# quentinll/pertrenderer

Hardware: AMD Instinct MI355X
Metric: rendered frames/sec + ms/backward, 256² img, 50 faces/px, 8 samples (higher is better)
Workload: dtype f32; 1 GPU; cfg2 pose-opt step: sphere_642 (1280 faces), 256x256, faces_per_pixel=50, Sr=Sa=8 Gaussian, sigma=1e-3 gamma=1e-2, blur=ln(1e4-1)*sigma, fwd + L2 loss (native) + bwd + Adam step on the pose (lr 5e-2); image_size=256, faces_per_pixel=50, nb_samples=8, rast_samples=8, batch=1, execution=graph, parallelism=single GPU

## Files before the change

pertrenderer_amd/csrc/pr_rast.hip:

```cpp
#include <cstdlib>
#include <type_traits>

#include <hip/hip_fp16.h>

#include "pr_common.h"

namespace pr {
namespace {

constexpr float kEps = 1e-8f;
constexpr int kTile = 4;

struct V2 {
  float x, y;
};

template <bool FAST = false>
PR_DEV float dv(float a, float b) {
  if constexpr (FAST) return a * __builtin_amdgcn_rcpf(b);
  else return a / b;
}

PR_DEV float edge_fn(V2 p, V2 a, V2 b) { return (p.x - a.x) * (b.y - a.y) - (p.y - a.y) * (b.x - a.x); }

// ... 256 lines not shown

template <bool PERSP, bool CLIP>
PR_DEV bool face_test(const FaceRec& r, V2 p, float blur, float& pz) {
  const bool inbox = !(p.x < r.c.y || p.x > r.c.z || p.y < r.c.w || p.y > r.d.x);
  float bc[3], d;
  bool inside;
  face_eval<PERSP, CLIP>(r, p, bc, pz, inside, d);
  return inbox && !(pz < 0.f) && (inside || d < blur);
}

PR_DEV float dist_margin(float4 ra, float4 rb, float ptile, float sqrt_blur, float blur) {
  const float m = fmaxf(fmaxf(fmaxf(fabsf(ra.x), fabsf(ra.y)), fmaxf(fabsf(ra.w), fabsf(rb.x))),
                        fmaxf(fmaxf(fabsf(rb.z), fabsf(rb.w)), ptile));
  const float delta = m * 0x1p-19f;
  return 4.f * sqrt_blur * delta + 2.f * delta * delta + blur * 0x1p-20f;
}

PR_DEV float seg_dist2_fast(V2 p, V2 a, float bax, float bay, float l2, V2 b) {
  const float bx = p.x - b.x, by = p.y - b.y;
  const float db = bx * bx + by * by;
  float t = (bax * (p.x - a.x) + bay * (p.y - a.y)) * __builtin_amdgcn_rcpf(l2);
  t = t < 0.f ? 0.f : (t > 1.f ? 1.f : t);
  const float qx = a.x + t * bax, qy = a.y + t * bay;
  const float dx = p.x - qx, dy = p.y - qy;
  const float ds = dx * dx + dy * dy;
  return l2 <= kEps ? db : ds;
}

PR_DEV bool face_maybe(const FaceRec& r, V2 p, float blur, float margin, float& dfast) {
  const bool inbox = !(p.x < r.c.y || p.x > r.c.z || p.y < r.c.w || p.y > r.d.x);
  const V2 v0{r.a.x, r.a.y}, v1{r.a.w, r.b.x}, v2{r.b.z, r.b.w};
  const float e0 = (p.x - v1.x) * r.e.w - (p.y - v1.y) * r.e.z;
  const float e1 = (p.x - v2.x) * r.f.y - (p.y - v2.y) * r.f.x;
  const float e2 = (p.x - v0.x) * r.e.y - (p.y - v0.y) * r.e.x;
  const bool pos = r.d.y > 0.f;
  const bool ins = e0 != 0.f && e1 != 0.f && e2 != 0.f && (e0 > 0.f) == pos && (e1 > 0.f) == pos &&
                   (e2 > 0.f) == pos;
  const float d01 = seg_dist2_fast(p, v0, r.e.x, r.e.y, r.d.z, v1);
  const float d02 = seg_dist2_fast(p, v0, -r.f.x, -r.f.y, r.f.z, v2);
  const float d12 = seg_dist2_fast(p, v1, r.e.z, r.e.w, r.d.w, v2);
  float d = d01 < d02 ? d01 : d02;
  d = d < d12 ? d : d12;
  dfast = d;
  return inbox && (ins || !(d > blur + margin));
}

template <bool CLIP>
PR_DEV bool face_test_kept(const FaceRec& r, V2 p, float blur, float margin, float dfast, float& pz) {
  const V2 v0{r.a.x, r.a.y}, v1{r.a.w, r.b.x}, v2{r.b.z, r.b.w};
  const float z0 = r.a.z, z1 = r.b.y, z2 = r.c.x;
  const float area = r.d.y;
  const float e0 = (p.x - v1.x) * r.e.w - (p.y - v1.y) * r.e.z;
  const float e1 = (p.x - v2.x) * r.f.y - (p.y - v2.y) * r.f.x;
  const float e2 = (p.x - v0.x) * r.e.y - (p.y - v0.y) * r.e.x;
  const float b[3] = {e0 / area, e1 / area, e2 / area};
  float bc[3];
  if constexpr (CLIP) {
    clip_fwd(b, bc);
  } else {
    bc[0] = b[0]; bc[1] = b[1]; bc[2] = b[2];
  }
  pz = bc[0] * z0 + bc[1] * z1 + bc[2] * z2;
  const bool inside = b[0] > 0.f && b[1] > 0.f && b[2] > 0.f;
  bool near = dfast < blur - margin;
  if (!inside && !near && !(dfast > blur + margin)) {
    const float d01 = seg_dist2_d(p, v0, r.e.x, r.e.y, r.d.z, v1);
    const float d02 = seg_dist2_d(p, v0, -r.f.x, -r.f.y, r.f.z, v2);
    const float d12 = seg_dist2_d(p, v1, r.e.z, r.e.w, r.d.w, v2);
    float d = d01 < d02 ? d01 : d02;
    d = d < d12 ? d : d12;
    near = d < blur;
  }
  return !(pz < 0.f) && (inside || near);
}

PR_DEV bool in_bbox(const FaceRec& r, V2 p) {
  return !(p.x < r.c.y || p.x > r.c.z || p.y < r.c.w || p.y > r.d.x);
}

#ifdef PR_RAST_PROFILE
constexpr unsigned kProfTiles = 1 << 16;
__device__ long long g_rast_prof[kProfTiles * 16];
#define PR_STAMP(i) (stamp[i] += (long long)__builtin_amdgcn_s_memtime() - t_, t_ = __builtin_amdgcn_s_memtime())
#else
#define PR_STAMP(i) ((void)0)
#endif

template <int SL> struct RastCfg {
  static constexpr int CAP = SL == 1 ? 512 : (SL == 2 ? 256 : 128);
#ifndef PR_RAST_G4
#define PR_RAST_G4 2
#endif
  static constexpr int G = SL == 1 ? 4 : (SL >= 4 ? PR_RAST_G4 : 2);
#ifndef PR_RAST_CH4
#define PR_RAST_CH4 16
#endif
  static constexpr int CH = SL >= 4 ? PR_RAST_CH4 : 64;
  static_assert(CAP <= 8 * 64, "suffix-min pass holds CAP / 64 <= 8 entries per lane");
};
#ifndef PR_RAST_QPAD
template <int SL> constexpr int rast_qpad() { return SL == 4 ? 1 : 0; }
#else
template <int SL> constexpr int rast_qpad() { return PR_RAST_QPAD; }
#endif
#ifndef PR_RAST_MERGE
#define PR_RAST_MERGE 1
#endif
#ifndef PR_RAST_FRAGC
#define PR_RAST_FRAGC 1
#endif
#ifndef PR_RAST_CULLU
#define PR_RAST_CULLU 16
#endif
constexpr int kCullU = PR_RAST_CULLU;
#ifndef PR_RAST_CHUNKU
#define PR_RAST_CHUNKU 16
#endif
constexpr int kChunkU = PR_RAST_CHUNKU;

template <int NT>
PR_DEV void bitonic_sort(float* key, int* val, int n2, int tid) {
  for (int k = 2; k <= n2; k <<= 1) {
    for (int j = k >> 1; j > 0; j >>= 1) {
      for (int i = tid; i < n2; i += NT) {
        const int ixj = i ^ j;
        if (ixj > i) {
          const bool up = (i & k) == 0;
          const float a = key[i], b = key[ixj];
          if ((a > b) == up) {
            key[i] = b; key[ixj] = a;
            const int t = val[i]; val[i] = val[ixj]; val[ixj] = t;
          }
        }
      }
      __syncthreads();
    }
  }
}

template <int E>
PR_DEV void wave_bitonic_sort(float (&key)[E], int (&val)[E], int lane) {
#pragma unroll
  for (int k = 2; k <= E * 64; k <<= 1) {
#pragma unroll
    for (int j = k >> 1; j > 0; j >>= 1) {
      if (j >= 64) {
        const int je = j >> 6;
#pragma unroll
        for (int e = 0; e < E; ++e) {
          const int pe = e ^ je;
          if (pe > e) {
            const bool up = ((e * 64 + lane) & k) == 0;
            const float a = key[e], b = key[pe];
            if ((a > b) == up) {
              key[e] = b; key[pe] = a;
              const int t = val[e]; val[e] = val[pe]; val[pe] = t;
            }
          }
        }
      } else {
#pragma unroll
        for (int e = 0; e < E; ++e) {
          const float ok = __shfl_xor(key[e], j);
          const int ov = __shfl_xor(val[e], j);
          const int i = e * 64 + lane;
          const bool up = (i & k) == 0, lower = (lane & j) == 0;
// ... 836 lines not shown
  gv[0] = g0; gv[1] = g1; gv[2] = g2;
}

PR_DEV void persp_bwd(const float b[3], float z0, float z1, float z2, const float go[3], float gb[3], float gz[3]) {
  const float t0 = b[0] * z1 * z2, t1 = z0 * b[1] * z2, t2 = z0 * z1 * b[2];
  const float s = t0 + t1 + t2;
  float gt[3];
  if (s > kEps) {
    const float is = __builtin_amdgcn_rcpf(s);
    const float dot = (go[0] * t0 + go[1] * t1 + go[2] * t2) * (is * is);
    gt[0] = go[0] * is - dot; gt[1] = go[1] * is - dot; gt[2] = go[2] * is - dot;
  } else {
    gt[0] = go[0] * 1e8f; gt[1] = go[1] * 1e8f; gt[2] = go[2] * 1e8f;
  }
  gb[0] = gt[0] * z1 * z2; gb[1] = gt[1] * z0 * z2; gb[2] = gt[2] * z0 * z1;
  gz[0] = gt[1] * b[1] * z2 + gt[2] * z1 * b[2];
  gz[1] = gt[0] * b[0] * z2 + gt[2] * z0 * b[2];
  gz[2] = gt[0] * b[0] * z1 + gt[1] * z0 * b[1];
}

PR_DEV void clip_bwd(const float b[3], const float go[3], float gb[3]) {
  const float w0 = b[0] > 0.f ? b[0] : 0.f, w1 = b[1] > 0.f ? b[1] : 0.f, w2 = b[2] > 0.f ? b[2] : 0.f;
  const float s = w0 + w1 + w2;
  float gw[3];
  if (s > 1e-5f) {
    const float is = __builtin_amdgcn_rcpf(s);
    const float dot = (go[0] * w0 + go[1] * w1 + go[2] * w2) * (is * is);
    gw[0] = go[0] * is - dot; gw[1] = go[1] * is - dot; gw[2] = go[2] * is - dot;
  } else {
    gw[0] = go[0] * 1e5f; gw[1] = go[1] * 1e5f; gw[2] = go[2] * 1e5f;
  }
  gb[0] = b[0] > 0.f ? gw[0] : 0.f;
  gb[1] = b[1] > 0.f ? gw[1] : 0.f;
  gb[2] = b[2] > 0.f ? gw[2] : 0.f;
}

PR_DEV void slot_grad(const PRRastArgs& a, V2 p, const float* v, int64_t o, float g[9]) {
  const V2 v0{v[0], v[1]}, v1{v[3], v[4]}, v2{v[6], v[7]};
  const float z0 = v[2], z1 = v[5], z2 = v[8];
  const bool persp = a.perspective_correct != 0, clip = a.clip_barycentric_coords != 0;
  const float gzb = a.grad_zbuf ? a.grad_zbuf[o] : 0.f;
  const float gd = a.grad_dists ? a.grad_dists[o] : 0.f;
  float gbu[3] = {0.f, 0.f, 0.f};
  if (a.grad_bary) { gbu[0] = a.grad_bary[o * 3]; gbu[1] = a.grad_bary[o * 3 + 1]; gbu[2] = a.grad_bary[o * 3 + 2]; }
  float bw[3], bp[3], bc[3];
  bary_fwd(p, v0, v1, v2, bw);
  if (persp) persp_fwd<true>(bw, z0, z1, z2, bp); else { bp[0] = bw[0]; bp[1] = bw[1]; bp[2] = bw[2]; }
  if (clip) clip_fwd<true>(bp, bc); else { bc[0] = bp[0]; bc[1] = bp[1]; bc[2] = bp[2]; }
  const bool inside = bp[0] > 0.f && bp[1] > 0.f && bp[2] > 0.f;
  V2 gdv[3];
  tri_dist2_bwd(p, v0, v1, v2, inside ? -gd : gd, gdv);
  float gsum[3] = {gbu[0] + gzb * z0, gbu[1] + gzb * z1, gbu[2] + gzb * z2};
  float gpp[3] = {gsum[0], gsum[1], gsum[2]};
  if (clip) clip_bwd(bp, gsum, gpp);
  float gw[3] = {gpp[0], gpp[1], gpp[2]};
  float gz[3] = {0.f, 0.f, 0.f};
  if (persp) persp_bwd(bw, z0, z1, z2, gpp, gw, gz);
  V2 gbv[3];
  bary_bwd(p, v0, v1, v2, gw, gbv);
  g[0] = gbv[0].x + gdv[0].x; g[1] = gbv[0].y + gdv[0].y; g[2] = gzb * bc[0] + gz[0];
  g[3] = gbv[1].x + gdv[1].x; g[4] = gbv[1].y + gdv[1].y; g[5] = gzb * bc[1] + gz[1];
  g[6] = gbv[2].x + gdv[2].x; g[7] = gbv[2].y + gdv[2].y; g[8] = gzb * bc[2] + gz[2];
}

PR_DEV void acc_edge(V2 p, V2 a, V2 b, float g, float* ga, float* gb) {
  ga[0] += g * (p.y - b.y); ga[1] += g * (b.x - p.x);
  gb[0] += g * (a.y - p.y); gb[1] += g * (p.x - a.x);
}

PR_DEV void acc_seg(V2 p, V2 a, V2 b, float g, float* ga, float* gb) {
  const float bax = b.x - a.x, bay = b.y - a.y;
  const float l2 = bax * bax + bay * bay;
  float t = 1.f;
  if (!(l2 <= kEps)) {
    t = (bax * (p.x - a.x) + bay * (p.y - a.y)) / l2;
    t = t < 0.f ? 0.f : (t > 1.f ? 1.f : t);
  }
  const float qx = (1.f - t) * a.x + t * b.x, qy = (1.f - t) * a.y + t * b.y;
  const float dx = qx - p.x, dy = qy - p.y;
  ga[0] += g * (1.f - t) * 2.f * dx; ga[1] += g * (1.f - t) * 2.f * dy;
  gb[0] += g * t * 2.f * dx;         gb[1] += g * t * 2.f * dy;
}

PR_DEV void slot_grad_exact(const PRRastArgs& a, V2 p, const float* v, int64_t o, float out[9]) {
  const V2 v0{v[0], v[1]}, v1{v[3], v[4]}, v2{v[6], v[7]};
  const float z0 = v[2], z1 = v[5], z2 = v[8];
  const bool persp = a.perspective_correct != 0, clip = a.clip_barycentric_coords != 0;
  const float gzb = a.grad_zbuf ? a.grad_zbuf[o] : 0.f;
  const float gd = a.grad_dists ? a.grad_dists[o] : 0.f;
  float gbu[3] = {0.f, 0.f, 0.f};
  if (a.grad_bary) { gbu[0] = a.grad_bary[o * 3]; gbu[1] = a.grad_bary[o * 3 + 1]; gbu[2] = a.grad_bary[o * 3 + 2]; }
  float bw[3], bp[3], bc[3];
  bary_fwd(p, v0, v1, v2, bw);
  if (persp) persp_fwd(bw, z0, z1, z2, bp); else { bp[0] = bw[0]; bp[1] = bw[1]; bp[2] = bw[2]; }
  if (clip) clip_fwd(bp, bc); else { bc[0] = bp[0]; bc[1] = bp[1]; bc[2] = bp[2]; }
  const bool inside = bp[0] > 0.f && bp[1] > 0.f && bp[2] > 0.f;
  float gv[3][2] = {{0.f, 0.f}, {0.f, 0.f}, {0.f, 0.f}};
  {
    const float g = inside ? -gd : gd;
    const float e01 = seg_dist2(p, v0, v1), e02 = seg_dist2(p, v0, v2), e12 = seg_dist2(p, v1, v2);
    if (e01 <= e02 && e01 <= e12) acc_seg(p, v0, v1, g, gv[0], gv[1]);
    else if (e02 <= e01 && e02 <= e12) acc_seg(p, v0, v2, g, gv[0], gv[2]);
    else acc_seg(p, v1, v2, g, gv[1], gv[2]);
  }
  const float gsum[3] = {gbu[0] + gzb * z0, gbu[1] + gzb * z1, gbu[2] + gzb * z2};
  float gpp[3] = {gsum[0], gsum[1], gsum[2]};
  if (clip) {
    const float w0 = bp[0] > 0.f ? bp[0] : 0.f, w1 = bp[1] > 0.f ? bp[1] : 0.f, w2 = bp[2] > 0.f ? bp[2] : 0.f;
    const float s = w0 + w1 + w2;
    float gw[3];
    if (s > 1e-5f) {
      const float dot = (gsum[0] * w0 + gsum[1] * w1 + gsum[2] * w2) / (s * s);
      gw[0] = gsum[0] / s - dot; gw[1] = gsum[1] / s - dot; gw[2] = gsum[2] / s - dot;
    } else {
      gw[0] = gsum[0] / 1e-5f; gw[1] = gsum[1] / 1e-5f; gw[2] = gsum[2] / 1e-5f;
    }
    gpp[0] = bp[0] > 0.f ? gw[0] : 0.f; gpp[1] = bp[1] > 0.f ? gw[1] : 0.f; gpp[2] = bp[2] > 0.f ? gw[2] : 0.f;
  }
  float gw[3] = {gpp[0], gpp[1], gpp[2]}, gzp[3] = {0.f, 0.f, 0.f};
  if (persp) {
    const float t0 = bw[0] * z1 * z2, t1 = z0 * bw[1] * z2, t2 = z0 * z1 * bw[2];
    const float s = t0 + t1 + t2;
    float gt[3];
    if (s > kEps) {
      const float dot = (gpp[0] * t0 + gpp[1] * t1 + gpp[2] * t2) / (s * s);
      gt[0] = gpp[0] / s - dot; gt[1] = gpp[1] / s - dot; gt[2] = gpp[2] / s - dot;
    } else {
      gt[0] = gpp[0] / kEps; gt[1] = gpp[1] / kEps; gt[2] = gpp[2] / kEps;
    }
    gw[0] = gt[0] * z1 * z2; gw[1] = gt[1] * z0 * z2; gw[2] = gt[2] * z0 * z1;
    gzp[0] = gt[1] * bw[1] * z2 + gt[2] * z1 * bw[2];
    gzp[1] = gt[0] * bw[0] * z2 + gt[2] * z0 * bw[2];
    gzp[2] = gt[0] * bw[0] * z1 + gt[1] * z0 * bw[1];
  }
  const float area = edge_fn(v2, v0, v1) + kEps;
  const float e0 = edge_fn(p, v1, v2), e1 = edge_fn(p, v2, v0), e2 = edge_fn(p, v0, v1);
  const float darea = -(gw[0] * e0 + gw[1] * e1 + gw[2] * e2) / (area * area);
  acc_edge(p, v1, v2, gw[0] / area, gv[1], gv[2]);
  acc_edge(p, v2, v0, gw[1] / area, gv[2], gv[0]);
  acc_edge(p, v0, v1, gw[2] / area, gv[0], gv[1]);
  gv[2][0] += darea * (v1.y - v0.y);
  gv[2][1] += darea * (v0.x - v1.x);
  acc_edge(v2, v0, v1, darea, gv[0], gv[1]);
#pragma unroll
  for (int i = 0; i < 3; ++i) {
    out[i * 3 + 0] = gv[i][0];
    out[i * 3 + 1] = gv[i][1];
    out[i * 3 + 2] = gzb * bc[i] + gzp[i];
  }
}

template <bool EXACT>
PR_DEV void slot_grad_any(const PRRastArgs& a, V2 p, const float* v, int64_t o, float g[9]) {
  if constexpr (EXACT) slot_grad_exact(a, p, v, o, g);
  else slot_grad(a, p, v, o, g);
}

__global__ void rast_bwd_keys_kernel(PRRastArgs a, uint32_t* keys, int64_t s0, int64_t n) {
  for (int64_t i = (int64_t)blockIdx.x * blockDim.x + threadIdx.x; i < n; i += (int64_t)gridDim.x * blockDim.x) {
    const int64_t o = s0 + i, pix = o / a.K;
    const bool valid = a.pix_count ? (int)(o - pix * a.K) < a.pix_count[pix] : true;
    const int64_t f = valid ? a.pix_to_face[o] : -1;
    keys[i] = f >= 0 ? (uint32_t)f : (uint32_t)a.F;
  }
}

__global__ void rast_bwd_sorted_grad_kernel(PRRastArgs a, const uint32_t* keys, const uint32_t* idx, float* vals,
                                            int64_t s0, int64_t n) {
  for (int64_t i = (int64_t)blockIdx.x * blockDim.x + threadIdx.x; i < n; i += (int64_t)gridDim.x * blockDim.x) {
    const uint32_t f = keys[i];
    if ((int64_t)f >= a.F) continue;
    const int64_t o = s0 + idx[i];
    const int64_t pix = o / a.K;
    const int col = (int)(pix % a.W), row = (int)((pix / a.W) % a.H);
    const V2 p{ndc(a.W - 1 - col, a.W, a.H), ndc(a.H - 1 - row, a.H, a.W)};
    float g[9];
    slot_grad_exact(a, p, a.face_verts + (int64_t)f * 9, o, g);
#pragma unroll
    for (int c = 0; c < 9; ++c) vals[i * 9 + c] = g[c];
  }
}

constexpr int kHash = 512;
constexpr int kBwdTile = 8;
constexpr int kBwdThreads = 256;
#ifndef PR_BWD_ENT
#define PR_BWD_ENT 512
#endif
constexpr int kBwdEnt = PR_BWD_ENT;
constexpr int kBwdFaces = 128;

template <int ROWS, bool EXACT>
__global__ void __launch_bounds__(kBwdThreads) rast_bwd_kernel(PRRastArgs a, int order) {
  constexpr int tile_rows = ROWS, TP = kBwdTile * ROWS;
  __shared__ int hkey[kHash];
  __shared__ int hfl[kHash];
  __shared__ int flist[kBwdFaces];
  __shared__ alignas(8) uint16_t M[kBwdFaces * TP];
  __shared__ float gbuf[9 * kBwdEnt];
  __shared__ int2 clist[kBwdEnt];
  __shared__ int ccount, nface;
  __shared__ float pxs[kBwdTile], pys[ROWS];
  __shared__ int pcnt[kBwdTile * ROWS];
  __shared__ int pstart[kBwdTile * ROWS + 1];
  const int tid = threadIdx.x, lane = tid & 63;
  const int K = a.K, H = a.H, W = a.W;
  const int n = blockIdx.z, col0 = blockIdx.x * kBwdTile;
  const int row0 = (order ? centre_out(blockIdx.y, gridDim.y) : (int)blockIdx.y) * tile_rows;
  const int ncols = min(kBwdTile, W - col0), nrows = min(tile_rows, H - row0);
  const int64_t tile_o = (((int64_t)n * H + row0) * W + col0) * K;
  const int64_t row_stride = (int64_t)W * K;
  for (int i = tid; i < kHash; i += kBwdThreads) hkey[i] = -1;
  for (int i = tid; i < kBwdFaces * TP; i += kBwdThreads) M[i] = 0xffff;
  if (tid < kBwdTile) pxs[tid] = ndc(W - 1 - min(col0 + tid, W - 1), W, H);
  if (tid >= 64 && tid < 64 + ROWS) pys[tid - 64] = ndc(H - 1 - min(row0 + tid - 64, H - 1), H, W);
  if (tid == 0) nface = 0;
  if (tid < TP) {
    const int r = tid / kBwdTile, c = tid - r * kBwdTile;
    pcnt[tid] = (r < nrows && c < ncols) ? (a.pix_count ? a.pix_count[((int64_t)n * H + row0 + r) * W + col0 + c] : K) : 0;
  }
  __syncthreads();
  if (tid == 0) {
    int acc_s = 0;
    for (int q = 0; q < TP; ++q) { pstart[q] = acc_s; acc_s += pcnt[q]; }
    pstart[TP] = acc_s;
  }
  __syncthreads();
  const int total = pstart[TP];
  float acc[9] = {0.f, 0.f, 0.f, 0.f, 0.f, 0.f, 0.f, 0.f, 0.f};
  for (int c0 = 0; c0 < total; c0 += kBwdEnt) {
    if (tid == 0) ccount = 0;
    __syncthreads();
    int64_t f[kBwdEnt / kBwdThreads];
    int pk[kBwdEnt / kBwdThreads];
#pragma unroll
    for (int u = 0; u < kBwdEnt / kBwdThreads; ++u) {
      const int i = c0 + u * kBwdThreads + tid;
      f[u] = -1;
      pk[u] = 0;
      if (i < total) {
        int q = 0;
#pragma unroll
        for (int step = TP / 2; step > 0; step >>= 1)
          if (pstart[q + step] <= i) q += step;
        const int k = i - pstart[q], r = q / kBwdTile, c = q - r * kBwdTile;
        pk[u] = (q << 16) | k;
        f[u] = a.pix_to_face[tile_o + r * row_stride + c * K + k];
      }
    }
#pragma unroll
    for (int u = 0; u < kBwdEnt / kBwdThreads; ++u) {
      const bool keep = f[u] >= 0;
      const uint64_t bal = __ballot(keep);
      if (bal == 0) continue;
      int off = 0;
      if (lane == 0) off = atomicAdd(&ccount, __popcll(bal));
      off = __shfl(off, 0);
      if (!keep) continue;
      const int fi = (int)f[u];
      clist[off + __popcll(bal & ((1ull << lane) - 1ull))] = make_int2(pk[u], fi);
      uint32_t h = ((uint32_t)fi * 2654435761u) & (kHash - 1);
      for (int probe = 0; probe < 32; ++probe) {
        const int cur = atomicCAS(&hkey[h], -1, fi);
        if (cur == -1) {
          const int fl = atomicAdd(&nface, 1);
          hfl[h] = fl;
          if (fl < kBwdFaces) flist[fl] = fi;
          break;
        }
        if (cur == fi) break;
        h = (h + 1) & (kHash - 1);
      }
    }
    __syncthreads();
    const int nv = ccount;
    for (int j = tid; j < nv; j += kBwdThreads) {
      const int2 e = clist[j];
      const int pix = e.x >> 16, k = e.x & 0xffff, fi = e.y;
      const int r = pix >> 3, c = pix & 7;
      const int64_t o = tile_o + r * row_stride + c * K + k;
      const V2 p{pxs[c], pys[r]};
      float g[9];
      slot_grad_any<EXACT>(a, p, a.face_verts + (int64_t)fi * 9, o, g);
      uint32_t h = ((uint32_t)fi * 2654435761u) & (kHash - 1);
      int fl = kBwdFaces;
      for (int probe = 0; probe < 32; ++probe) {
        const int cur = hkey[h];
        if (cur == fi) { fl = hfl[h]; break; }
        if (cur == -1) break;
        h = (h + 1) & (kHash - 1);
      }
      if (fl < kBwdFaces) {
#pragma unroll
        for (int cc = 0; cc < 9; ++cc) gbuf[cc * kBwdEnt + j] = g[cc];
        M[((pix >> 2) * kBwdFaces + fl) * 4 + (pix & 3)] = (uint16_t)j;
      } else {
#pragma unroll
        for (int cc = 0; cc < 9; ++cc) atomicAdd(&a.grad_face_verts[(int64_t)fi * 9 + cc], g[cc]);
      }
    }
    __syncthreads();
    if (tid < min(nface, kBwdFaces)) {
      uint64_t* col = reinterpret_cast<uint64_t*>(M) + tid;
      for (int q = 0; q < nrows * kBwdTile; q += 4) {
        const uint64_t four = col[(q >> 2) * kBwdFaces];
        if (four == ~0ull) continue;
        col[(q >> 2) * kBwdFaces] = ~0ull;
#pragma unroll
        for (int t = 0; t < 4; ++t) {
          const uint32_t jj = (uint32_t)(four >> (16 * t)) & 0xffffu;
          if (jj == 0xffffu) continue;
#pragma unroll
          for (int cc = 0; cc < 9; ++cc) acc[cc] += gbuf[cc * kBwdEnt + jj];
        }
      }
    }
  }
  __syncthreads();
  const int nf = min(nface, kBwdFaces);
  if (tid < nf) {
#pragma unroll
    for (int cc = 0; cc < 9; ++cc) gbuf[tid * 9 + cc] = acc[cc];
  }
  __syncthreads();
  for (int i = tid; i < nf * 9; i += kBwdThreads) {
    const int fl = i / 9, cc = i - fl * 9;
    atomicAdd(&a.grad_face_verts[(int64_t)flist[fl] * 9 + cc], gbuf[i]);
  }
}

PR_DEV int64_t attr_row(const PRInterpArgs& a, int64_t f, int i) {
  return a.faces ? a.faces[f * 3 + i] * a.D : (f * 3 + i) * a.D;
}

__global__ void interp_fwd_kernel(PRInterpArgs a) {
  for (int64_t s = (int64_t)blockIdx.x * blockDim.x + threadIdx.x; s < a.PK; s += (int64_t)gridDim.x * blockDim.x) {
    const int64_t f = a.pix_to_face[s];
    float* o = a.out + s * a.D;
    if (f < 0) {
      for (int d = 0; d < a.D; ++d) o[d] = 0.f;
      continue;
    }
    const float w0 = a.bary[s * 3], w1 = a.bary[s * 3 + 1], w2 = a.bary[s * 3 + 2];
    const float* r0 = a.face_attr + attr_row(a, f, 0);
    const float* r1 = a.face_attr + attr_row(a, f, 1);
    const float* r2 = a.face_attr + attr_row(a, f, 2);
    for (int d = 0; d < a.D; ++d) o[d] = (w0 * r0[d] + w1 * r1[d]) + w2 * r2[d];
  }
}

__global__ void interp_bwd_kernel(PRInterpArgs a) {
  for (int64_t s = (int64_t)blockIdx.x * blockDim.x + threadIdx.x; s < a.PK; s += (int64_t)gridDim.x * blockDim.x) {
    const int64_t f = a.pix_to_face[s];
    const float* go = a.grad_out + s * a.D;
    if (f < 0) {
      if (a.grad_bary) { a.grad_bary[s * 3] = 0.f; a.grad_bary[s * 3 + 1] = 0.f; a.grad_bary[s * 3 + 2] = 0.f; }
      continue;
    }
    const float w[3] = {a.bary[s * 3], a.bary[s * 3 + 1], a.bary[s * 3 + 2]};
    const int64_t rows[3] = {attr_row(a, f, 0), attr_row(a, f, 1), attr_row(a, f, 2)};
    float gb[3] = {0.f, 0.f, 0.f};
    for (int d = 0; d < a.D; ++d) {
      const float g = go[d];
#pragma unroll
      for (int i = 0; i < 3; ++i) {
        gb[i] += g * a.face_attr[rows[i] + d];
        if (a.grad_face_attr && g != 0.f) atomicAdd(&a.grad_face_attr[rows[i] + d], w[i] * g);
      }
    }
    if (a.grad_bary) { a.grad_bary[s * 3] = gb[0]; a.grad_bary[s * 3 + 1] = gb[1]; a.grad_bary[s * 3 + 2] = gb[2]; }
  }
}

PR_DEV int mesh_of(const int64_t* first, const int64_t* nf, int N, int64_t f) {
  for (int n = 0; n < N; ++n)
    if (f >= first[n] && f < first[n] + nf[n]) return n;
  return 0;
}

PR_DEV void xform(const float* M, float x, float y, float z, float o[4]) {
#pragma unroll
  for (int c = 0; c < 4; ++c) o[c] = ((x * M[c] + y * M[4 + c]) + z * M[8 + c]) + M[12 + c];
}

__global__ void project_fwd_kernel(PRProjectArgs a) {
  for (int64_t t = (int64_t)blockIdx.x * blockDim.x + threadIdx.x; t < a.F * 3; t += (int64_t)gridDim.x * blockDim.x) {
    const int64_t f = t / 3;
    const int n = mesh_of(a.mesh_first_face, a.mesh_num_faces, a.N, f);
    const float* v = a.verts + a.faces[t] * 3;
    float o[4], c[4];
    xform(a.world_to_view + n * 16, v[0], v[1], v[2], o);
    const float vx = o[0] / o[3], vy = o[1] / o[3], vz = o[2] / o[3];
    xform(a.proj + n * 16, vx, vy, vz, c);
    a.face_verts[t * 3 + 0] = c[0] / c[3];
    a.face_verts[t * 3 + 1] = c[1] / c[3];
    a.face_verts[t * 3 + 2] = vz;
  }
}

__global__ void project_prep_kernel(PRProjectArgs a, float blur_v, const float* blur_dev, int cull_backfaces,
                                    FaceRec* recs, uint2* bbox, float* zero_fv, float* zero_v, BinGrid bins) {
  const int64_t stride = (int64_t)gridDim.x * blockDim.x;
  const float blur = blur_dev ? *blur_dev : blur_v;
  if (a.seed_advance && blockIdx.x == 0 && threadIdx.x == 0) {
    const unsigned i = threadIdx.x;
    uint64_t s = a.seed_advance[i];
    for (int k = 0; k < a.seed_advance_n; ++k) s = seed_next(s);
    a.seed_advance[i] = s;
  }
  for (int64_t f0 = (int64_t)blockIdx.x * blockDim.x + (threadIdx.x & ~63u); f0 < a.F; f0 += stride) {
    const int64_t f = f0 + (threadIdx.x & 63u);
// ... 60 lines not shown
      for (int64_t j0 = s; j0 < e; j0 += kGatherB) {
        int64_t t[kGatherB];
#pragma unroll
        for (int u = 0; u < kGatherB; ++u) t[u] = j0 + u < e ? a.vert_corners[j0 + u] : -1;
        if (j0 == s) t0 = t[0];
        float c[kGatherB][3];
#pragma unroll
        for (int u = 0; u < kGatherB; ++u) {
          if (t[u] >= 0) {
            c[u][0] = a.grad_face_verts[t[u] * 3];
            c[u][1] = a.grad_face_verts[t[u] * 3 + 1];
            c[u][2] = a.grad_face_verts[t[u] * 3 + 2];
          }
        }
#pragma unroll
        for (int u = 0; u < kGatherB; ++u) {
          if (t[u] >= 0) {
            gx += c[u][0];
            gy += c[u][1];
            gz += c[u][2];
          }
        }
      }
      const int n = mesh_of(a.mesh_first_face, a.mesh_num_faces, a.N, t0 / 3);
      project_vertex_bwd(a.world_to_view + n * 16, a.proj + n * 16, a.verts + vi * 3, gx, gy, gz, g);
    }
    a.grad_verts[vi * 3] = g[0];
    a.grad_verts[vi * 3 + 1] = g[1];
    a.grad_verts[vi * 3 + 2] = g[2];
  }
}

__global__ void project_bwd_kernel(PRProjectArgs a) {
  for (int64_t t = (int64_t)blockIdx.x * blockDim.x + threadIdx.x; t < a.F * 3; t += (int64_t)gridDim.x * blockDim.x) {
    const int64_t f = t / 3;
    const int n = mesh_of(a.mesh_first_face, a.mesh_num_faces, a.N, f);
    const int64_t vi = a.faces[t];
    const float* v = a.verts + vi * 3;
    const float* M = a.world_to_view + n * 16;
    const float* P = a.proj + n * 16;
    float o[4], c[4];
    xform(M, v[0], v[1], v[2], o);
    const float vv[3] = {o[0] / o[3], o[1] / o[3], o[2] / o[3]};
    xform(P, vv[0], vv[1], vv[2], c);
    const float gx = a.grad_face_verts[t * 3], gy = a.grad_face_verts[t * 3 + 1], gz = a.grad_face_verts[t * 3 + 2];
    const float i3 = 1.f / c[3], i33 = i3 * i3;
    float gvv[3];
#pragma unroll
    for (int k = 0; k < 3; ++k) {
      gvv[k] = gx * (P[k * 4 + 0] * i3 - c[0] * P[k * 4 + 3] * i33) + gy * (P[k * 4 + 1] * i3 - c[1] * P[k * 4 + 3] * i33);
    }
    gvv[2] += gz;
    const float j3 = 1.f / o[3], j33 = j3 * j3;
#pragma unroll
    for (int m = 0; m < 3; ++m) {
      float g = 0.f;
#pragma unroll
      for (int k = 0; k < 3; ++k) g += gvv[k] * (M[m * 4 + k] * j3 - o[k] * M[m * 4 + 3] * j33);
      atomicAdd(&a.grad_verts[vi * 3 + m], g);
    }
  }
}

int rast_check(const PRRastArgs& a) {
  if (a.N <= 0 || a.H <= 0 || a.W <= 0 || a.K <= 0) return set_error(PR_ERR_ARG, "rast: bad shape");
  if (a.F < 0 || a.F >= (int64_t(1) << 31)) return set_error(PR_ERR_ARG, "rast: face count out of range");
  if (!a.face_verts && a.F > 0) return set_error(PR_ERR_ARG, "rast: face_verts missing");
  if (!a.mesh_first_face || !a.mesh_num_faces) return set_error(PR_ERR_ARG, "rast: mesh index missing");
  if (a.K > 512) return set_error(PR_ERR_ARG, "rast: faces_per_pixel must be <= 512");
  if ((int64_t)a.H > 65535 || (int64_t)a.W > 65535 * kTile || a.N > 65535)
    return set_error(PR_ERR_ARG, "rast: image too large");
  return PR_OK;
}

}
}

using namespace pr;

#ifdef PR_RAST_PROFILE
extern "C" int pr_rast_prof_dump(void* dst, size_t bytes) {
  return hipMemcpyFromSymbol(dst, HIP_SYMBOL(g_rast_prof), bytes < sizeof(g_rast_prof) ? bytes : sizeof(g_rast_prof),
                             0, hipMemcpyDeviceToHost) == hipSuccess ? 0 : -1;
}
#endif

static BinGrid bin_grid(const PRRastArgs& a, void* ws) {
  BinGrid g{};
  g.H = a.H; g.W = a.W;
  if (a.bin_size <= 0 || a.N <= 0 || a.H <= 0 || a.W <= 0) return g;
  g.bs = (a.bin_size + 7) / 8 * 8;
  g.nx = (a.W + g.bs - 1) / g.bs;
  g.ny = (a.H + g.bs - 1) / g.bs;
  const int64_t F = a.F > 0 ? a.F : 1;
  const int64_t mfpb = a.max_faces_per_bin > 0 ? a.max_faces_per_bin : std::max<int64_t>(10000, F / 5);
  g.cap = (int)std::min<int64_t>(mfpb, F);
  if (ws) {
    char* p = reinterpret_cast<char*>(ws) + (size_t)F * (sizeof(FaceRec) + sizeof(uint2));
    g.count = reinterpret_cast<int*>(p);
    g.list = g.count + (size_t)a.N * g.ny * g.nx;
  }
  return g;
}

static size_t bin_bytes(const PRRastArgs& a) {
  const BinGrid g = bin_grid(a, nullptr);
  if (g.bs == 0) return 0;
  const size_t nb = (size_t)a.N * g.ny * g.nx;
  return nb * sizeof(int) * (1 + (size_t)g.cap);
}

extern "C" size_t pr_rast_fwd_workspace_size(const PRRastArgs* a) {
  if (!a) return 0;
  return (size_t)(a->F > 0 ? a->F : 1) * (sizeof(FaceRec) + sizeof(uint2)) + bin_bytes(*a);
}

static int bins_begin(const PRRastArgs& a, BinGrid& g, hipStream_t st) {
  g = bin_grid(a, a.workspace);
  if (!g.count) return PR_OK;
  if (hipMemsetAsync(g.count, 0, (size_t)a.N * g.ny * g.nx * sizeof(int), st) != hipSuccess)
    return set_error(PR_ERR_HIP, "rast_fwd: bin counter memset failed");
  return PR_OK;
}

static int rast_fwd_prepared(const PRRastArgs& a, const FaceRec* fr, const uint2* fbox, const BinGrid& bins,
                             hipStream_t st);

extern "C" int pr_rast_fwd(const PRRastArgs* args, void* stream) {
  if (!args) return set_error(PR_ERR_ARG, "rast_fwd: null args");
  const PRRastArgs& a = *args;
  if (int e = rast_check(a)) return e;
  if (!a.pix_to_face || !a.zbuf || !a.bary || !a.dists) return set_error(PR_ERR_ARG, "rast_fwd: output missing");
  if (!a.workspace || a.workspace_bytes < pr_rast_fwd_workspace_size(args))
    return set_error(PR_ERR_WORKSPACE, "rast_fwd: workspace too small");
  hipStream_t st = reinterpret_cast<hipStream_t>(stream);
  FaceRec* fr = reinterpret_cast<FaceRec*>(a.workspace);
  uint2* fbox = reinterpret_cast<uint2*>(fr + (a.F > 0 ? a.F : 1));
  BinGrid bins;
  if (int e = bins_begin(a, bins, st)) return e;
  if (a.F > 0) {
    const int nb = (int)std::min<int64_t>((a.F + kThreads - 1) / kThreads, 1024);
    face_prep_kernel<<<nb, kThreads, 0, st>>>(a.face_verts, a.F, a.blur_radius, a.blur_radius_dev, a.cull_backfaces, fr,
                                              fbox, bins, a.mesh_first_face, a.N);
    if (int e = check_launch("rast_face_prep")) return e;
  }
  return rast_fwd_prepared(a, fr, fbox, bins, st);
}

static int rast_fwd_prepared(const PRRastArgs& a, const FaceRec* fr, const uint2* fbox, const BinGrid& bins,
                             hipStream_t st) {
  int sl = (int64_t)a.K * 16 * 8 > 16 * 1024 ? 8 : 4;
  if (const char* e = getenv("PR_RAST_SLICES")) {
    const int v = atoi(e);
    if (v == 1 || v == 2 || v == 4 || v == 8) sl = v;
  }
  bool frag = true;
  if (const char* e = getenv("PR_RAST_FRAG")) frag = atoi(e) != 0;
  const char* duo = getenv("PR_RAST_DUO");
  const int nw = sl == 4 && duo && duo[0] == '1' ? 2 : 1;
  size_t lds = rast_fwd_lds(a.K, sl, nw);
  if (const char* e = getenv("PR_RAST_LDS_MIN")) lds = std::max(lds, (size_t)atol(e));
  if (lds > 160 * 1024) return set_error(PR_ERR_ARG, "rast_fwd: faces_per_pixel too large for the LDS queue (max 300)");
  const char* cc = getenv("PR_RAST_CHUNK_CULL");
  const int chunk_cull = !(cc && cc[0] == '0');
  launch_rast_fwd(a, fr, fbox, chunk_cull, sl, frag, lds, bins, st, nw);
  if (int e = check_launch("rast_fwd")) return e;
// ... 150 lines not shown
```

Baseline: 3773 frames/s (fwd+bwd).

## Restructure raster backward: skip zero-dist-grad work, store hash slots, split reductions

Reworks the rasterizer backward kernel in several ways. Slots whose grad_dists is zero are partitioned to the back of the candidate list so the edge-distance gradient can be skipped for them, guarded by a finiteness check on the vertices. The hash slot is stored in a packed clist entry so the second hash probe is avoided. The pixel-count prefix sum now uses wave shuffles, and empty tiles exit early. The per-face accumulation is split across two thread halves with shared partial sums, and the hash and entry sizes are halved with an occupancy hint to reduce LDS use and raise occupancy. Tile columns are also rotated, and profiling hooks are added. Risks include more rounds per tile because of the smaller entry buffer, and the packed 10-bit fields limiting K and the hash size.

```diff
diff --git a/pertrenderer_amd/csrc/pr_rast.hip b/pertrenderer_amd/csrc/pr_rast.hip
--- a/pertrenderer_amd/csrc/pr_rast.hip
+++ b/pertrenderer_amd/csrc/pr_rast.hip
@@ -362,6 +362,7 @@
 constexpr unsigned kProfTiles = 1 << 16;
 __device__ long long g_rast_prof[kProfTiles * 16];
 #define PR_STAMP(i) (stamp[i] += (long long)__builtin_amdgcn_s_memtime() - t_, t_ = __builtin_amdgcn_s_memtime())
+__device__ long long g_rast_bwd_prof[kProfTiles * 16];
 #else
 #define PR_STAMP(i) ((void)0)
 #endif
@@ -1364,27 +1365,31 @@
   gb[0] += g * t * 2.f * dx;         gb[1] += g * t * 2.f * dy;
 }
 
-PR_DEV void slot_grad_exact(const PRRastArgs& a, V2 p, const float* v, int64_t o, float out[9]) {
+PR_DEV void slot_grad_exact(const PRRastArgs& a, V2 p, const float* v, int64_t o, float out[9], bool gd_zero = false) {
   const V2 v0{v[0], v[1]}, v1{v[3], v[4]}, v2{v[6], v[7]};
   const float z0 = v[2], z1 = v[5], z2 = v[8];
   const bool persp = a.perspective_correct != 0, clip = a.clip_barycentric_coords != 0;
-  const float gzb = a.grad_zbuf ? a.grad_zbuf[o] : 0.f;
-  const float gd = a.grad_dists ? a.grad_dists[o] : 0.f;
-  float gbu[3] = {0.f, 0.f, 0.f};
-  if (a.grad_bary) { gbu[0] = a.grad_bary[o * 3]; gbu[1] = a.grad_bary[o * 3 + 1]; gbu[2] = a.grad_bary[o * 3 + 2]; }
   float bw[3], bp[3], bc[3];
   bary_fwd(p, v0, v1, v2, bw);
   if (persp) persp_fwd(bw, z0, z1, z2, bp); else { bp[0] = bw[0]; bp[1] = bw[1]; bp[2] = bw[2]; }
   if (clip) clip_fwd(bp, bc); else { bc[0] = bp[0]; bc[1] = bp[1]; bc[2] = bp[2]; }
   const bool inside = bp[0] > 0.f && bp[1] > 0.f && bp[2] > 0.f;
   float gv[3][2] = {{0.f, 0.f}, {0.f, 0.f}, {0.f, 0.f}};
-  {
+  constexpr float kTame = 1e9f;
+  const bool tame = fabsf(v0.x) < kTame && fabsf(v0.y) < kTame && fabsf(v1.x) < kTame && fabsf(v1.y) < kTame &&
+                    fabsf(v2.x) < kTame && fabsf(v2.y) < kTame && fabsf(z0) < INFINITY && fabsf(z1) < INFINITY &&
+                    fabsf(z2) < INFINITY;
+  if (!(gd_zero && tame)) {
+    const float gd = a.grad_dists ? a.grad_dists[o] : 0.f;
     const float g = inside ? -gd : gd;
     const float e01 = seg_dist2(p, v0, v1), e02 = seg_dist2(p, v0, v2), e12 = seg_dist2(p, v1, v2);
     if (e01 <= e02 && e01 <= e12) acc_seg(p, v0, v1, g, gv[0], gv[1]);
     else if (e02 <= e01 && e02 <= e12) acc_seg(p, v0, v2, g, gv[0], gv[2]);
     else acc_seg(p, v1, v2, g, gv[1], gv[2]);
   }
+  const float gzb = a.grad_zbuf ? a.grad_zbuf[o] : 0.f;
+  float gbu[3] = {0.f, 0.f, 0.f};
+  if (a.grad_bary) { gbu[0] = a.grad_bary[o * 3]; gbu[1] = a.grad_bary[o * 3 + 1]; gbu[2] = a.grad_bary[o * 3 + 2]; }
   const float gsum[3] = {gbu[0] + gzb * z0, gbu[1] + gzb * z1, gbu[2] + gzb * z2};
   float gpp[3] = {gsum[0], gsum[1], gsum[2]};
   if (clip) {
@@ -1463,71 +1468,135 @@
   }
 }
 
-constexpr int kHash = 512;
+constexpr int kHash = 256;
 constexpr int kBwdTile = 8;
 constexpr int kBwdThreads = 256;
 #ifndef PR_BWD_ENT
-#define PR_BWD_ENT 512
+#define PR_BWD_ENT 256
+#endif
+#ifndef PR_BWD_WAVES
+#define PR_BWD_WAVES 6
 #endif
 constexpr int kBwdEnt = PR_BWD_ENT;
 constexpr int kBwdFaces = 128;
+constexpr int kBwdSplit = kBwdThreads / kBwdFaces;
+#ifndef PR_BWD_ROT
+#define PR_BWD_ROT 5
+#endif
+constexpr unsigned kBwdRot = PR_BWD_ROT;
+constexpr uint32_t kBwdNoHash = 1023;
+static_assert(kBwdEnt % kBwdThreads == 0 && kBwdEnt <= 65535, "round size");
+static_assert(kHash <= (int)kBwdNoHash, "hash slot field");
+
+#ifdef PR_RAST_PROFILE
+PR_DEV void bwd_prof_record(long long rt0, const long long* stamp, int tile_x, int tile_y, int total, int rounds, int nface,
+                            const int* pcount) {
+  unsigned hw, xcc;
+  asm volatile("s_getreg_b32 %0, hwreg(HW_REG_HW_ID)" : "=s"(hw));
+  asm volatile("s_getreg_b32 %0, hwreg(HW_REG_XCC_ID)" : "=s"(xcc));
+  const unsigned t = (blockIdx.z * gridDim.y + blockIdx.y) * gridDim.x + blockIdx.x;
+  if (t >= kProfTiles) return;
+  long long* rec = g_rast_bwd_prof + (size_t)t * 16;
+  rec[0] = tile_x; rec[1] = tile_y; rec[2] = blockIdx.z; rec[3] = total;
+  rec[4] = rt0; rec[5] = (long long)__builtin_amdgcn_s_memrealtime();
+  rec[6] = (long long)hw | ((long long)(xcc & 0xf) << 32);
+  for (int i = 0; i < 5; ++i) rec[7 + i] = stamp[i];
+  rec[12] = rounds; rec[13] = nface;
+  rec[14] = (long long)pcount[0] | ((long long)pcount[1] << 32);
+  rec[15] = (long long)pcount[2] | ((long long)pcount[3] << 32);
+}
+#endif
 
 template <int ROWS, bool EXACT>
-__global__ void __launch_bounds__(kBwdThreads) rast_bwd_kernel(PRRastArgs a, int order) {
+__global__ void __launch_bounds__(kBwdThreads, PR_BWD_WAVES) rast_bwd_kernel(PRRastArgs a, int order) {
   constexpr int tile_rows = ROWS, TP = kBwdTile * ROWS;
+  static_assert(TP <= 64, "one wave scans the pixel counts; the clist pixel field has 6 bits");
   __shared__ int hkey[kHash];
   __shared__ int hfl[kHash];
   __shared__ int flist[kBwdFaces];
   __shared__ alignas(8) uint16_t M[kBwdFaces * TP];
   __shared__ float gbuf[9 * kBwdEnt];
-  __shared__ int2 clist[kBwdEnt];
-  __shared__ int ccount, nface;
+  __shared__ float sums[9 * kBwdThreads];
+  __shared__ uint32_t clist[kBwdEnt];
+  __shared__ int cfront, cback, nface;
   __shared__ float pxs[kBwdTile], pys[ROWS];
-  __shared__ int pcnt[kBwdTile * ROWS];
   __shared__ int pstart[kBwdTile * ROWS + 1];
   const int tid = threadIdx.x, lane = tid & 63;
   const int K = a.K, H = a.H, W = a.W;
-  const int n = blockIdx.z, col0 = blockIdx.x * kBwdTile;
+  const int n = blockIdx.z;
+  const int tile_x = order ? (int)((blockIdx.x + kBwdRot * (blockIdx.y >> 3)) % gridDim.x) : (int)blockIdx.x;
+  const int col0 = tile_x * kBwdTile;
   const int row0 = (order ? centre_out(blockIdx.y, gridDim.y) : (int)blockIdx.y) * tile_rows;
   const int ncols = min(kBwdTile, W - col0), nrows = min(tile_rows, H - row0);
   const int64_t tile_o = (((int64_t)n * H + row0) * W + col0) * K;
   const int64_t row_stride = (int64_t)W * K;
+#ifdef PR_RAST_PROFILE
+  __shared__ int pcount[4];
+  long long stamp[5] = {0, 0, 0, 0, 0}, t_ = __builtin_amdgcn_s_memtime();
+  const long long rt0 = __builtin_amdgcn_s_memrealtime();
+  int rounds = 0;
+  if (tid < 4) pcount[tid] = 0;
+#endif
+  if (tid < 64) {
+    int cnt = 0;
+    if (tid < TP) {
+      const int r = tid / kBwdTile, c = tid - r * kBwdTile;
+      if (r < nrows && c < ncols) cnt = a.pix_count ? a.pix_count[((int64_t)n * H + row0 + r) * W + col0 + c] : K;
+    }
+    int incl = cnt;
+#pragma unroll
+    for (int d = 1; d < TP; d <<= 1) {
+      const int up = __shfl_up(incl, d);
+      if (lane >= d) incl += up;
+    }
+    if (tid < TP) pstart[tid] = incl - cnt;
+    if (tid == TP - 1) pstart[TP] = incl;
+  }
+  __syncthreads();
+  const int total = pstart[TP];
+  if (total == 0) {
+#ifdef PR_RAST_PROFILE
+    PR_STAMP(0);
+    if (tid == 0) bwd_prof_record(rt0, stamp, tile_x, row0 / tile_rows, 0, 0, 0, pcount);
+#endif
+    return;
+  }
   for (int i = tid; i < kHash; i += kBwdThreads) hkey[i] = -1;
   for (int i = tid; i < kBwdFaces * TP; i += kBwdThreads) M[i] = 0xffff;
   if (tid < kBwdTile) pxs[tid] = ndc(W - 1 - min(col0 + tid, W - 1), W, H);
   if (tid >= 64 && tid < 64 + ROWS) pys[tid - 64] = ndc(H - 1 - min(row0 + tid - 64, H - 1), H, W);
   if (tid == 0) nface = 0;
-  if (tid < TP) {
-    const int r = tid / kBwdTile, c = tid - r * kBwdTile;
-    pcnt[tid] = (r < nrows && c < ncols) ? (a.pix_count ? a.pix_count[((int64_t)n * H + row0 + r) * W + col0 + c] : K) : 0;
-  }
-  __syncthreads();
-  if (tid == 0) {
-    int acc_s = 0;
-    for (int q = 0; q < TP; ++q) { pstart[q] = acc_s; acc_s += pcnt[q]; }
-    pstart[TP] = acc_s;
-  }
-  __syncthreads();
-  const int total = pstart[TP];
-  float acc[9] = {0.f, 0.f, 0.f, 0.f, 0.f, 0.f, 0.f, 0.f, 0.f};
+#pragma unroll
+  for (int cc = 0; cc < 9; ++cc) sums[cc * kBwdThreads + tid] = 0.f;
+  const int own_fl = tid % kBwdFaces, own_part = tid / kBwdFaces;
+  PR_STAMP(0);
   for (int c0 = 0; c0 < total; c0 += kBwdEnt) {
-    if (tid == 0) ccount = 0;
+    if (tid == 0) { cfront = 0; cback = 0; }
     __syncthreads();
+    PR_STAMP(3);
+#ifdef PR_RAST_PROFILE
+    ++rounds;
+#endif
     int64_t f[kBwdEnt / kBwdThreads];
     int pk[kBwdEnt / kBwdThreads];
+    bool front[kBwdEnt / kBwdThreads];
 #pragma unroll
     for (int u = 0; u < kBwdEnt / kBwdThreads; ++u) {
       const int i = c0 + u * kBwdThreads + tid;
       f[u] = -1;
       pk[u] = 0;
+      front[u] = false;
       if (i < total) {
         int q = 0;
 #pragma unroll
         for (int step = TP / 2; step > 0; step >>= 1)
           if (pstart[q + step] <= i) q += step;
         const int k = i - pstart[q], r = q / kBwdTile, c = q - r * kBwdTile;
-        pk[u] = (q << 16) | k;
-        f[u] = a.pix_to_face[tile_o + r * row_stride + c * K + k];
+        const int64_t o = tile_o + r * row_stride + c * K + k;
+        pk[u] = (q << 10) | k;
+        f[u] = a.pix_to_face[o];
+        if constexpr (EXACT) front[u] = a.grad_dists ? a.grad_dists[o] != 0.f : false;
+        else front[u] = true;
       }
     }
 #pragma unroll
@@ -1535,43 +1604,68 @@
       const bool keep = f[u] >= 0;
       const uint64_t bal = __ballot(keep);
       if (bal == 0) continue;
-      int off = 0;
-      if (lane == 0) off = atomicAdd(&ccount, __popcll(bal));
-      off = __shfl(off, 0);
+      const uint64_t balf = __ballot(keep && front[u]), balb = bal & ~balf;
+      int offf = 0, offb = 0;
+      if (lane == 0) {
+        if (balf) offf = atomicAdd(&cfront, __popcll(balf));
+        if (balb) offb = atomicAdd(&cback, __popcll(balb));
+      }
+      offf = __shfl(offf, 0);
+      offb = __shfl(offb, 0);
       if (!keep) continue;
       const int fi = (int)f[u];
-      clist[off + __popcll(bal & ((1ull << lane) - 1ull))] = make_int2(pk[u], fi);
-      uint32_t h = ((uint32_t)fi * 2654435761u) & (kHash - 1);
+      uint32_t h = ((uint32_t)fi * 2654435761u) & (kHash - 1), hs = kBwdNoHash;
       for (int probe = 0; probe < 32; ++probe) {
         const int cur = atomicCAS(&hkey[h], -1, fi);
         if (cur == -1) {
           const int fl = atomicAdd(&nface, 1);
           hfl[h] = fl;
           if (fl < kBwdFaces) flist[fl] = fi;
+          hs = h;
           break;
         }
-        if (cur == fi) break;
+        if (cur == fi) { hs = h; break; }
         h = (h + 1) & (kHash - 1);
       }
+      const uint64_t below = (1ull << lane) - 1ull;
+      const int pos = front[u] ? offf + __popcll(balf & below) : kBwdEnt - 1 - (offb + __popcll(balb & below));
+      clist[pos] = ((uint32_t)pk[u] << 10) | hs;
     }
     __syncthreads();
-    const int nv = ccount;
-    for (int j = tid; j < nv; j += kBwdThreads) {
-      const int2 e = clist[j];
-      const int pix = e.x >> 16, k = e.x & 0xffff, fi = e.y;
+    PR_STAMP(1);
+    const int nfr = cfront, nv = nfr + cback;
+#pragma unroll
+    for (int u = 0; u < kBwdEnt / kBwdThreads; ++u) {
+      const int jj = u * kBwdThreads + tid;
+      if (jj >= nv) break;
+      const bool with_dist = jj < nfr;
+      const int j = with_dist ? jj : jj + (kBwdEnt - nv);
+      const uint32_t e = clist[j];
+      const int pix = e >> 20, k = (e >> 10) & 1023;
+      const uint32_t hs = e & 1023;
       const int r = pix >> 3, c = pix & 7;
       const int64_t o = tile_o + r * row_stride + c * K + k;
+      int fi, fl = kBwdFaces;
+      if (hs != kBwdNoHash) { fi = hkey[hs]; fl = hfl[hs]; }
+      else fi = (int)a.pix_to_face[o];
+#ifdef PR_RAST_PROFILE
+      {
+        const bool nz = a.grad_zbuf && a.grad_zbuf[o] != 0.f, nd = a.grad_dists && a.grad_dists[o] != 0.f;
+        const bool nb = a.grad_bary && (a.grad_bary[o * 3] != 0.f || a.grad_bary[o * 3 + 1] != 0.f ||
+                                        a.grad_bary[o * 3 + 2] != 0.f);
+        const uint64_t bz = __ballot(nz), bd = __ballot(nd), bb = __ballot(nb), bn = __ballot(!nz && !nd && !nb);
+        if (lane == __ffsll((unsigned long long)__ballot(true)) - 1) {
+          atomicAdd(&pcount[0], __popcll(bz));
+          atomicAdd(&pcount[1], __popcll(bd));
+          atomicAdd(&pcount[2], __popcll(bb));
+          atomicAdd(&pcount[3], __popcll(bn));
+        }
+      }
+#endif
       const V2 p{pxs[c], pys[r]};
       float g[9];
-      slot_grad_any<EXACT>(a, p, a.face_verts + (int64_t)fi * 9, o, g);
-      uint32_t h = ((uint32_t)fi * 2654435761u) & (kHash - 1);
-      int fl = kBwdFaces;
-      for (int probe = 0; probe < 32; ++probe) {
-        const int cur = hkey[h];
-        if (cur == fi) { fl = hfl[h]; break; }
-        if (cur == -1) break;
-        h = (h + 1) & (kHash - 1);
-      }
+      if constexpr (EXACT) slot_grad_exact(a, p, a.face_verts + (int64_t)fi * 9, o, g, !with_dist);
+      else slot_grad(a, p, a.face_verts + (int64_t)fi * 9, o, g);
       if (fl < kBwdFaces) {
 #pragma unroll
         for (int cc = 0; cc < 9; ++cc) gbuf[cc * kBwdEnt + j] = g[cc];
@@ -1582,12 +1676,16 @@
       }
     }
     __syncthreads();
-    if (tid < min(nface, kBwdFaces)) {
-      uint64_t* col = reinterpret_cast<uint64_t*>(M) + tid;
-      for (int q = 0; q < nrows * kBwdTile; q += 4) {
-        const uint64_t four = col[(q >> 2) * kBwdFaces];
+    PR_STAMP(2);
+    if (own_fl < min(nface, kBwdFaces)) {
+      uint64_t* col = reinterpret_cast<uint64_t*>(M) + own_fl;
+      float acc[9];
+#pragma unroll
+      for (int cc = 0; cc < 9; ++cc) acc[cc] = sums[cc * kBwdThreads + tid];
+      for (int q4 = own_part; q4 < nrows * (kBwdTile / 4); q4 += kBwdSplit) {
+        const uint64_t four = col[q4 * kBwdFaces];
         if (four == ~0ull) continue;
-        col[(q >> 2) * kBwdFaces] = ~0ull;
+        col[q4 * kBwdFaces] = ~0ull;
 #pragma unroll
         for (int t = 0; t < 4; ++t) {
           const uint32_t jj = (uint32_t)(four >> (16 * t)) & 0xffffu;
@@ -1596,19 +1694,25 @@
           for (int cc = 0; cc < 9; ++cc) acc[cc] += gbuf[cc * kBwdEnt + jj];
         }
       }
+#pragma unroll
+      for (int cc = 0; cc < 9; ++cc) sums[cc * kBwdThreads + tid] = acc[cc];
     }
   }
   __syncthreads();
+  PR_STAMP(3);
   const int nf = min(nface, kBwdFaces);
-  if (tid < nf) {
-#pragma unroll
-    for (int cc = 0; cc < 9; ++cc) gbuf[tid * 9 + cc] = acc[cc];
-  }
-  __syncthreads();
   for (int i = tid; i < nf * 9; i += kBwdThreads) {
     const int fl = i / 9, cc = i - fl * 9;
-    atomicAdd(&a.grad_face_verts[(int64_t)flist[fl] * 9 + cc], gbuf[i]);
-  }
+    float s = sums[cc * kBwdThreads + fl];
+#pragma unroll
+    for (int part = 1; part < kBwdSplit; ++part) s += sums[cc * kBwdThreads + part * kBwdFaces + fl];
+    atomicAdd(&a.grad_face_verts[(int64_t)flist[fl] * 9 + cc], s);
+  }
+#ifdef PR_RAST_PROFILE
+  __syncthreads();
+  PR_STAMP(4);
+  if (tid == 0) bwd_prof_record(rt0, stamp, tile_x, row0 / tile_rows, total, rounds, nface, pcount);
+#endif
 }
 
 PR_DEV int64_t attr_row(const PRInterpArgs& a, int64_t f, int i) {
@@ -1835,6 +1939,11 @@
 extern "C" int pr_rast_prof_dump(void* dst, size_t bytes) {
   return hipMemcpyFromSymbol(dst, HIP_SYMBOL(g_rast_prof), bytes < sizeof(g_rast_prof) ? bytes : sizeof(g_rast_prof),
                              0, hipMemcpyDeviceToHost) == hipSuccess ? 0 : -1;
+}
+extern "C" int pr_rast_bwd_prof_dump(void* dst, size_t bytes) {
+  return hipMemcpyFromSymbol(dst, HIP_SYMBOL(g_rast_bwd_prof),
+                             bytes < sizeof(g_rast_bwd_prof) ? bytes : sizeof(g_rast_bwd_prof), 0,
+                             hipMemcpyDeviceToHost) == hipSuccess ? 0 : -1;
 }
 #endif
 
```

Measured after the change: 3843 frames/s (fwd+bwd) (median of 6 runs). 1.8% higher.
